# LLNL/saamge

Hardware: AMD Instinct MI355X
Metric: AMG setup+solve DoF/s (3D Poisson, PCG to 1e-8) (higher is better)
Workload: dtype f64; 1 GPU; 3D Poisson 256^3 Q1 hexes, 3-level SAAMGE, theta=0.003, nu_relax=3, 8x8x4-element AEs, 8x8x4-AE coarse blocks; workload_id=poisson256, dofs=16974593, converged=True, parallelism=single GPU

## Files before the change

### saamge_amd/csrc/mis.hip

```cpp
#include "mis.h"
#include "assemble.h"

#include <cfloat>

namespace saamge_amd {

__device__ inline double wsum(double v) {
#pragma unroll
    for (int o = 32; o > 0; o >>= 1) v += __shfl_xor(v, o, 64);
    return v;
}

__global__ __launch_bounds__(64) void mis_svd_kernel(
    const int *__restrict__ mis2d_I, const int *__restrict__ mis2d_J,
    const int *__restrict__ mis2ae_I, const int *__restrict__ mis2ae_J,
    const int *__restrict__ ae2d_I, const int64_t *__restrict__ pair_loc_off,
    const int *__restrict__ pair_loc, const signed char *__restrict__ flags, MisSvdIO io, int m0,
    const int *__restrict__ list = nullptr) {
    extern __shared__ __align__(16) double lds[];
    const int m = list ? list[blockIdx.x] : m0 + (int)blockIdx.x;
    const int lane = threadIdx.x;
    const int r = mis2d_I[m + 1] - mis2d_I[m];
    const int *dofs = mis2d_J + mis2d_I[m];
    double *M = io.gather + io.g_off[m];
// ... 309 lines not shown
        hipLaunchKernelGGL(mis_copy_kernel, dim3(div_up(nm, 4)), dim3(256), 0, s, v, nm, rep.p);
        SA_HIP_CHECK(hipGetLastError());
        SA_HIP_CHECK(hipStreamSynchronize(s));
        profiler().end(s, "mis_svd", 0.0, 0.0);
        return;
    }
    profiler().begin(s);
    hipLaunchKernelGGL(mis_svd_kernel, dim3(num_mises), dim3(64), lds, s, rel.mis2d_I.p,
                       rel.mis2d_J.p, rel.mis2ae_I.p, rel.mis2ae_J.p, rel.ae2d_I.p,
                       rel.pair_loc_off.p, rel.pair_loc.p, rel.flags.p, io, m0);
    SA_HIP_CHECK(hipGetLastError());
    profiler().end(s, "mis_svd", 0.0, 0.0);
}

__global__ __launch_bounds__(256) void p_count_kernel(int ND, const int *__restrict__ mises,
                                                      const int *__restrict__ k, int *__restrict__ cnt) {
    const long i = (long)blockIdx.x * 256 + threadIdx.x;
    if (i < ND) cnt[i] = k[mises[i]];
}

__global__ __launch_bounds__(256) void r_len_kernel(int nm, const int *__restrict__ mis2d_I, const int *__restrict__ k,
                                                    const int *__restrict__ coloff, int *__restrict__ len) {
    const int m = blockIdx.x * 256 + threadIdx.x;
    if (m >= nm) return;
    const int r = mis2d_I[m + 1] - mis2d_I[m], c0 = coloff[m];
    for (int v = 0; v < k[m]; ++v) len[c0 + v] = r;
}

template <class OUT>
__global__ __launch_bounds__(256) void scan_tile_kernel(int n, const int *__restrict__ in,
                                                        OUT *__restrict__ out, OUT *__restrict__ tsum) {
    __shared__ OUT sh[256];
    const long base = (long)blockIdx.x * 1024;
    int v[4];
    OUT run = 0;
    for (int q = 0; q < 4; ++q) {
        const long i = base + threadIdx.x * 4 + q;
        v[q] = (i < n) ? in[i] : 0;
        run += v[q];
    }
    sh[threadIdx.x] = run;
    __syncthreads();
    for (int o = 1; o < 256; o <<= 1) {
        const OUT t = (threadIdx.x >= o) ? sh[threadIdx.x - o] : 0;
        __syncthreads();
        sh[threadIdx.x] += t;
        __syncthreads();
    }
    OUT excl = sh[threadIdx.x] - run;
    for (int q = 0; q < 4; ++q) {
        const long i = base + threadIdx.x * 4 + q;
        if (i < n) out[i] = excl;
        excl += v[q];
    }
    if (threadIdx.x == 255) tsum[blockIdx.x] = sh[255];
}
template <class OUT>
__global__ __launch_bounds__(256) void scan_sums_kernel(int nt, OUT *__restrict__ tsum, OUT *__restrict__ total) {
    __shared__ OUT sh[256];
    __shared__ OUT carry;
    if (threadIdx.x == 0) carry = 0;
    __syncthreads();
    for (int base = 0; base < nt; base += 256) {
        const int i = base + threadIdx.x;
        const OUT x = (i < nt) ? tsum[i] : 0;
        sh[threadIdx.x] = x;
        __syncthreads();
        for (int o = 1; o < 256; o <<= 1) {
            const OUT t = (threadIdx.x >= o) ? sh[threadIdx.x - o] : 0;
            __syncthreads();
            sh[threadIdx.x] += t;
            __syncthreads();
        }
        if (i < nt) tsum[i] = carry + sh[threadIdx.x] - x;
        __syncthreads();
        if (threadIdx.x == 255) carry += sh[255];
        __syncthreads();
    }
    if (threadIdx.x == 0) *total = carry;
}
template <class OUT>
__global__ __launch_bounds__(256) void scan_add_kernel(int n, OUT *__restrict__ out,
                                                       const OUT *__restrict__ tsum,
                                                       const OUT *__restrict__ total) {
    const long i = (long)blockIdx.x * 256 + threadIdx.x;
    if (i < n) out[i] += tsum[i >> 10];
    if (i == 0) out[n] = *total;
}

template <class OUT>
static void exclusive_scan_t(hipStream_t s, int n, const int *in, OUT *out) {
    const int nt = div_up(n, 1024);
    DBuf<OUT> tsum((size_t)nt + 1);
    hipLaunchKernelGGL(scan_tile_kernel<OUT>, dim3(nt), dim3(256), 0, s, n, in, out, tsum.p);
    hipLaunchKernelGGL(scan_sums_kernel<OUT>, dim3(1), dim3(256), 0, s, nt, tsum.p, tsum.p + nt);
    hipLaunchKernelGGL(scan_add_kernel<OUT>, dim3(div_up(n, 256)), dim3(256), 0, s, n, out, (const OUT *)tsum.p, (const OUT *)(tsum.p + nt));
    SA_HIP_CHECK(hipGetLastError());
    SA_HIP_CHECK(hipStreamSynchronize(s));
}
void exclusive_scan_int(hipStream_t s, int n, const int *in, int *out) { exclusive_scan_t<int>(s, n, in, out); }
void exclusive_scan_int_async(hipStream_t s, int n, const int *in, int *out, int *tsum) {
    const int nt = div_up(n, 1024);
    hipLaunchKernelGGL(scan_tile_kernel<int>, dim3(nt), dim3(256), 0, s, n, in, out, tsum);
    hipLaunchKernelGGL(scan_sums_kernel<int>, dim3(1), dim3(256), 0, s, nt, tsum, tsum + nt);
    hipLaunchKernelGGL(scan_add_kernel<int>, dim3(div_up(n, 256)), dim3(256), 0, s, n, out, (const int *)tsum, (const int *)(tsum + nt));
    SA_HIP_CHECK(hipGetLastError());
}
void exclusive_scan_off(hipStream_t s, int n, const int *in, roff_t *out) { exclusive_scan_t<roff_t>(s, n, in, out); }

__global__ __launch_bounds__(256) void p_fill_kernel(int ND, const int *__restrict__ mises,
                                                     const int *__restrict__ row_in_mis,
                                                     const int *__restrict__ mis2d_I,
                                                     const int *__restrict__ k,
                                                     const int *__restrict__ coloff,
                                                     const int64_t *__restrict__ u_off,
                                                     const double *__restrict__ U,
                                                     const roff_t *__restrict__ rowptr,
                                                     int *__restrict__ col, double *__restrict__ val) {
    const long i = (long)blockIdx.x * 256 + threadIdx.x;
    if (i >= ND) return;
    const int m = mises[i], km = k[m];
    const int r = mis2d_I[m + 1] - mis2d_I[m];
    const double *Um = U + u_off[m] + row_in_mis[i];
    const roff_t base = rowptr[i];
    const int c0 = coloff[m];
    for (int v = 0; v < km; ++v) {
        col[base + v] = c0 + v;
        val[base + v] = Um[(size_t)v * r];
    }
}

__global__ __launch_bounds__(256) void r_fill_kernel(int num_mises, const int *__restrict__ mis2d_I,
                                                     const int *__restrict__ mis2d_J,
                                                     const int *__restrict__ k,
                                                     const int *__restrict__ coloff,
                                                     const int64_t *__restrict__ u_off,
                                                     const double *__restrict__ U,
                                                     const roff_t *__restrict__ rowptr,
                                                     int *__restrict__ col, double *__restrict__ val) {
    const int m = blockIdx.x;
    const int km = k[m];
    if (km == 0) return;
    const int r = mis2d_I[m + 1] - mis2d_I[m];
    const int *dofs = mis2d_J + mis2d_I[m];
    const double *Um = U + u_off[m];
    for (int idx = threadIdx.x; idx < km * r; idx += 256) {
        const int v = idx / r, i = idx % r;
        const roff_t base = rowptr[coloff[m] + v];
        col[base + i] = dofs[i];
        val[base + i] = Um[(size_t)v * r + i];
    }
}

void build_P_R(hipStream_t s, const DevRelations &rel, const Relations &hrel,
               const std::vector<int> &h_k, const std::vector<int64_t> &h_u_off, const int *d_k,
               const int *d_coloff, const int64_t *d_u_off, const double *U, DCsr &P, DCsr &R) {
    (void)h_u_off;
    const int ND = hrel.ND;
    int nc = 0;
    int64_t nnz = 0;
    for (int m = 0; m < hrel.num_mises; ++m) {
        nc += h_k[m];
        nnz += (int64_t)h_k[m] * hrel.mis_to_dof.row_size(m);
    }
    P.nrows = ND; P.ncols = nc; P.nnz = nnz;
    P.rowptr.alloc((size_t)ND + 1);
    P.col.alloc((size_t)nnz);
    P.val.alloc((size_t)nnz);
    {
        DBuf<int> cnt((size_t)ND);
        hipLaunchKernelGGL(p_count_kernel, dim3(div_up(ND, 256)), dim3(256), 0, s, ND, rel.mises.p, d_k, cnt.p);
        exclusive_scan_off(s, ND, cnt.p, P.rowptr.p);
    }
    hipLaunchKernelGGL(p_fill_kernel, dim3(div_up(ND, 256)), dim3(256), 0, s, ND, rel.mises.p,
                       rel.dof_row_in_mis.p, rel.mis2d_I.p, d_k, d_coloff, d_u_off, U, P.rowptr.p,
                       P.col.p, P.val.p);
    P.lanes_per_row = pick_lanes_per_row(nnz, ND);
    R.nrows = nc; R.ncols = ND; R.nnz = nnz;
    {
        DBuf<int> len((size_t)std::max(nc, 1));
        R.rowptr.alloc((size_t)nc + 1);
        if (hrel.num_mises)
            hipLaunchKernelGGL(r_len_kernel, dim3(div_up(hrel.num_mises, 256)), dim3(256), 0, s, hrel.num_mises, rel.mis2d_I.p, d_k,
                               d_coloff, len.p);
        if (nc > 0) exclusive_scan_off(s, nc, len.p, R.rowptr.p);
        else SA_HIP_CHECK(hipMemsetAsync(R.rowptr.p, 0, sizeof(roff_t), s));
    }
    R.col.alloc((size_t)nnz);
    R.val.alloc((size_t)nnz);
    if (hrel.num_mises)
        hipLaunchKernelGGL(r_fill_kernel, dim3(hrel.num_mises), dim3(256), 0, s, hrel.num_mises,
                           rel.mis2d_I.p, rel.mis2d_J.p, d_k, d_coloff, d_u_off, U, R.rowptr.p,
                           R.col.p, R.val.p);
    SA_HIP_CHECK(hipGetLastError());
    R.lanes_per_row = pick_lanes_per_row(nnz, nc > 0 ? nc : 1);
}

__global__ __launch_bounds__(256) void ae_mis_k_kernel(long n, const int *__restrict__ ae2mis_J,
                                                       const int *__restrict__ k, int *__restrict__ out) {
    const long i = (long)blockIdx.x * 256 + threadIdx.x;
    if (i < n) out[i] = k[ae2mis_J[i]];
}

__global__ __launch_bounds__(256) void ae_ke_max_kernel(int nparts, const int *__restrict__ ae2mis_I,
                                                        const int *__restrict__ colpos_ptr, int *__restrict__ out) {
    const int e = blockIdx.x * 256 + threadIdx.x;
    int ke = 0;
    if (e < nparts) ke = colpos_ptr[ae2mis_I[e + 1]] - colpos_ptr[ae2mis_I[e]];
#pragma unroll
    for (int o = 32; o > 0; o >>= 1) ke = max(ke, __shfl_xor(ke, o, 64));
    if ((threadIdx.x & 63) == 0) atomicMax(out, ke);
}

__global__ __launch_bounds__(256) void coarse_e2d_kernel(
    const int *__restrict__ ae2d_I, const int *__restrict__ ae2d_J, const int *__restrict__ ae2mis_I,
    const int *__restrict__ ae2mis_J, const int *__restrict__ mises, const int *__restrict__ mis_k,
    const int *__restrict__ mis_coloff, const int *__restrict__ colpos_ptr, const roff_t *__restrict__ prow,
    const double *__restrict__ pval, int cap, int *__restrict__ colpos, int *__restrict__ e2d_J,
    int *__restrict__ err) {
    extern __shared__ unsigned long long ce_keys[];
    int *cd = (int *)(ce_keys + cap);
    const int e = blockIdx.x, tid = threadIdx.x;
    const int tb = ae2mis_I[e], te = ae2mis_I[e + 1];
    const int c0 = colpos_ptr[tb], KE = colpos_ptr[te] - c0;
    for (int t = tb + tid; t < te; t += 256) {
        const int m = ae2mis_J[t], km = mis_k[m], base = colpos_ptr[t] - c0, co = mis_coloff[m];
        for (int v = 0; v < km; ++v) {
            ce_keys[base + v] = ~0ull;
            cd[base + v] = co + v;
        }
    }
    __syncthreads();
    const int d0 = ae2d_I[e], d1 = ae2d_I[e + 1];
    for (int k = d0 + tid; k < d1; k += 256) {
        const int dof = ae2d_J[k], m = mises[dof], km = mis_k[m];
        if (km == 0) continue;
        int lo = tb, hi = te;
        while (lo < hi) {
            const int mid = (lo + hi) >> 1;
            if (ae2mis_J[mid] < m) lo = mid + 1; else hi = mid;
        }
        const int base = colpos_ptr[lo] - c0;
        const roff_t pr = prow[dof];
        for (int v = 0; v < km; ++v)
            if (pval[pr + v] != 0.0)
                atomicMin(&ce_keys[base + v], ((unsigned long long)(unsigned)(k - d0) << 32) | (unsigned)(base + v));
    }
    __syncthreads();
    for (int idx = tid; idx < KE; idx += 256) {
        const unsigned long long key = ce_keys[idx];
        if (key == ~0ull) {
            colpos[c0 + idx] = -1;
            atomicExch(err, 1);
            continue;
        }
        int rank = 0;
        for (int j = 0; j < KE; ++j) rank += (ce_keys[j] < key) ? 1 : 0;
        colpos[c0 + idx] = rank;
        e2d_J[c0 + rank] = cd[idx];
    }
}

bool coarse_e2d_device(hipStream_t s, const DevRelations &rel, const Relations &hrel, const int *d_mis_k,
                       const int *d_mis_coloff, int ncoarse, const roff_t *p_rowptr, const double *p_val,
                       DBuf<int> &colpos_ptr, DBuf<int> &colpos, Table &e2d) {
    const int nparts = hrel.nparts;
    const long npairs = (long)hrel.AE_to_mis.J.size();
    if (nparts == 0 || npairs == 0) return false;
    DBuf<int> kk((size_t)npairs), info(2);
    info.zero(s);
    hipLaunchKernelGGL(ae_mis_k_kernel, dim3(div_up(npairs, 256)), dim3(256), 0, s, npairs, rel.ae2mis_J.p, d_mis_k, kk.p);
    colpos_ptr.alloc((size_t)npairs + 1);
    exclusive_scan_int(s, (int)npairs, kk.p, colpos_ptr.p);
    hipLaunchKernelGGL(ae_ke_max_kernel, dim3(div_up(nparts, 256)), dim3(256), 0, s, nparts, rel.ae2mis_I.p, colpos_ptr.p, info.p);
    SA_HIP_CHECK(hipGetLastError());
    const int cap = info.to_host(s)[0];
    const size_t lds = (size_t)cap * 12 + 16;
    if (lds > 60 * 1024) return false;
    auto h_ptr = colpos_ptr.to_host(s);
    const int total = h_ptr[(size_t)npairs];
    colpos.alloc((size_t)total + 1);
    DBuf<int> d_J((size_t)total + 1);
    if (total) {
        hipLaunchKernelGGL(coarse_e2d_kernel, dim3(nparts), dim3(256), lds, s, rel.ae2d_I.p, rel.ae2d_J.p, rel.ae2mis_I.p,
                           rel.ae2mis_J.p, rel.mises.p, d_mis_k, d_mis_coloff, colpos_ptr.p, p_rowptr, p_val, cap, colpos.p,
                           d_J.p, info.p + 1);
        SA_HIP_CHECK(hipGetLastError());
    }
    SA_REQUIRE(info.to_host(s)[1] == 0, "coarse dof with an all-zero prolongator column in an AE");
    e2d.ncols = ncoarse;
    e2d.I.resize((size_t)nparts + 1);
    for (int e = 0; e <= nparts; ++e) e2d.I[e] = h_ptr[(size_t)hrel.AE_to_mis.I[e]];
    e2d.J.resize((size_t)total);
    if (total) {
        SA_HIP_CHECK(hipMemcpyAsync(e2d.J.data(), d_J.p, sizeof(int) * (size_t)total, hipMemcpyDeviceToHost, s));
        SA_HIP_CHECK(hipStreamSynchronize(s));
    }
    return true;
}

constexpr int RAP_NT = 256;
constexpr int RAP_HASH = 2048;
constexpr int RAP_SMALL_ROWS = 64;

template <int NT, int CAP>
__global__ __launch_bounds__(NT) void rap_symbolic_kernel(
    const int *__restrict__ mlist, int pass, const int *__restrict__ mis2d_I, const int *__restrict__ mis2d_J,
    const roff_t *__restrict__ Arow, const int *__restrict__ Acol, const int *__restrict__ mises,
    const int *__restrict__ k, int *__restrict__ cnt, const int *__restrict__ nbr_ptr,
    int *__restrict__ nbr, int *__restrict__ err, int *__restrict__ stage = nullptr, int stage_cap = 0,
    int maxrow = 0) {
    __shared__ int table[CAP];
    __shared__ int nfound;
    const int m1 = mlist ? mlist[blockIdx.x] : (int)blockIdx.x;
    if (k[m1] == 0) {
        if (pass == 0 && threadIdx.x == 0) cnt[m1] = 0;
        return;
    }
    const int r1 = mis2d_I[m1 + 1] - mis2d_I[m1];
    const int *dofs = mis2d_J + mis2d_I[m1];
    __shared__ int overflow;
    int HS = CAP;
    if (maxrow > 0) {
        const long bound = 2l * r1 * maxrow;
        HS = 64;
        while (HS < 256 && HS < bound) HS <<= 1;
    }
    const bool certain = maxrow > 0 && 2l * r1 * maxrow <= HS;
    for (;;) {
        for (int i = threadIdx.x; i < HS; i += NT) table[i] = -1;
        if (threadIdx.x == 0) { nfound = 0; overflow = 0; }
        __syncthreads();
        for (int il = threadIdx.x; il < r1; il += NT) {
            const int g = dofs[il];
            for (roff_t q = Arow[g]; q < Arow[g + 1]; ++q) {
                const int m2 = mises[Acol[q]];
                if (k[m2] == 0) continue;
                unsigned h = hash_home((unsigned)m2, (unsigned)HS);
                for (int probe = 0; probe < HS; ++probe) {
                    const int old = atomicCAS(&table[h], -1, m2);
                    if (old == -1) { atomicAdd(&nfound, 1); break; }
                    if (old == m2) break;
                    h = (h + 1) & (HS - 1);
                    if (probe == HS - 1) { if (HS == RAP_HASH) atomicExch(err, 1); else overflow = 1; }
                }
            }
        }
        __syncthreads();
        const bool full = !certain && (overflow || 2 * nfound > HS);
        const bool again = HS < CAP && full;
        __syncthreads();
        if (CAP < RAP_HASH && full && !again) {
            if (threadIdx.x == 0) cnt[m1] = -1;
            return;
        }
        if (!again) break;
        HS = CAP;
    }
    if (pass == 0) {
        if (threadIdx.x == 0) cnt[m1] = nfound;
        if (!stage || nfound > stage_cap) return;
    }
    __shared__ int list[CAP];
    __shared__ int nlist;
    if (threadIdx.x == 0) nlist = 0;
    __syncthreads();
    for (int i = threadIdx.x; i < HS; i += NT) {
        const int v = table[i];
        if (v >= 0) list[atomicAdd(&nlist, 1)] = v;
    }
    __syncthreads();
    const int nl = nlist;
    int *out = (pass == 0) ? stage + (size_t)m1 * stage_cap : nbr + nbr_ptr[m1];
    for (int i = threadIdx.x; i < nl; i += NT) {
        const int v = list[i];
        int rank = 0;
        for (int j = 0; j < nl; ++j) rank += (list[j] < v);
        out[rank] = v;
    }
}

__global__ __launch_bounds__(256) void rap_unstage_kernel(int nm, int cap, const int *__restrict__ stage,
                                                          const int *__restrict__ nbr_ptr, int *__restrict__ nbr) {
    const long i = (long)blockIdx.x * 256 + threadIdx.x;
    const int m = (int)(i / cap), t = (int)(i % cap);
    if (m < nm && t < nbr_ptr[m + 1] - nbr_ptr[m]) nbr[nbr_ptr[m] + t] = stage[i];
}

template <int NT>
__global__ __launch_bounds__(NT) void rap_numeric_kernel(
    const int *__restrict__ list, int m_first, const int *__restrict__ mis2d_I, const int *__restrict__ mis2d_J, const roff_t *__restrict__ Arow,
    const int *__restrict__ Acol, const double *__restrict__ Aval, const int *__restrict__ mises,
    const int *__restrict__ row_in_mis, const int *__restrict__ k, const int *__restrict__ coloff,
    const int64_t *__restrict__ u_off, const double *__restrict__ U,
    const int *__restrict__ nbr_ptr, const int *__restrict__ nbr, const roff_t *__restrict__ crowptr,
    int *__restrict__ ccol, double *__restrict__ cval, int lds_doubles) {
    extern __shared__ __align__(16) double lds[];
    const int m1 = list ? list[blockIdx.x] : m_first + (int)blockIdx.x;
    const int k1 = k[m1];
    if (k1 == 0) return;
    const int tid = threadIdx.x;
    const int nn = nbr_ptr[m1 + 1] - nbr_ptr[m1];
    const int *nb = nbr + nbr_ptr[m1];
    const int r1 = mis2d_I[m1 + 1] - mis2d_I[m1];
    const int *dofs = mis2d_J + mis2d_I[m1];
    const double *U1 = U + u_off[m1];
    const int pos_d = 3 * nn + 2;
    long long *uo = (long long *)lds;
    int *pos = (int *)(uo + nn);
    int *nbl = pos + nn + 1;
    int *kk = nbl + nn;
    int *rr = kk + nn;
    for (int t = tid; t < nn; t += NT) {
        const int m2 = nb[t];
        nbl[t] = m2;
        kk[t] = k[m2];
        rr[t] = mis2d_I[m2 + 1] - mis2d_I[m2];
        uo[t] = u_off[m2];
    }
    __syncthreads();
    if (tid == 0) {
        int run = 0;
        for (int t = 0; t < nn; ++t) { pos[t] = run; run += kk[t]; }
        pos[nn] = run;
    }
    __syncthreads();
    const int ncol = pos[nn];
    double *acc = lds + pos_d;
    const int rows_total = (lds_doubles - pos_d) / ncol;
    const int KC = (k1 + 1 <= rows_total) ? k1 : rows_total / 2;
    const int RC = rows_total - KC;
    double *T = acc + (size_t)KC * ncol;
    for (int idx = tid; idx < k1 * ncol; idx += NT) {
        const int v1 = idx / ncol, cc = idx % ncol;
        int lo = 0, hi = nn;
        while (hi - lo > 1) { const int mid = (lo + hi) >> 1; if (pos[mid] <= cc) lo = mid; else hi = mid; }
        ccol[crowptr[coloff[m1] + v1] + cc] = coloff[nbl[lo]] + (cc - pos[lo]);
    }
    for (int v0 = 0; v0 < k1; v0 += KC) {
        const int kc = min(KC, k1 - v0);
        __syncthreads();
        for (int i = tid; i < kc * ncol; i += NT) acc[i] = 0.0;
        for (int c0 = 0; c0 < r1; c0 += RC) {
            const int rc = min(RC, r1 - c0);
            __syncthreads();
            for (int i = tid; i < rc * ncol; i += NT) T[i] = 0.0;
            __syncthreads();
            for (int il = tid; il < rc; il += NT) {
                const int g = dofs[c0 + il];
                double *Trow = T + (size_t)il * ncol;
                const roff_t qe = Arow[g + 1];
                for (roff_t q0 = Arow[g]; q0 < qe; q0 += 4) {
                    int jj4[4], lo4[4];
                    double a4[4], u4[4];
                    bool on4[4];
#pragma unroll
                    for (int t = 0; t < 4; ++t) {
                        const roff_t q = min(q0 + t, qe - 1);
                        jj4[t] = Acol[q];
                        a4[t] = Aval[q];
                    }
                    int m4[4], rim4[4];
#pragma unroll
                    for (int t = 0; t < 4; ++t) { m4[t] = mises[jj4[t]]; rim4[t] = row_in_mis[jj4[t]]; }
#pragma unroll
                    for (int t = 0; t < 4; ++t) {
                        int lo = 0, hi = nn;
                        while (hi - lo > 1) { const int mid = (lo + hi) >> 1; if (nbl[mid] <= m4[t]) lo = mid; else hi = mid; }
                        lo4[t] = lo;
                        on4[t] = q0 + t < qe && nn != 0 && nbl[lo] == m4[t];
                        u4[t] = on4[t] ? U[uo[lo] + rim4[t]] : 0.0;
                    }
#pragma unroll
                    for (int t = 0; t < 4; ++t) {
                        if (!on4[t]) continue;
                        const int lo = lo4[t];
                        const int k2 = kk[lo];
                        const int r2 = rr[lo];
                        const double *U2 = U + uo[lo] + rim4[t];
                        double *dst = Trow + pos[lo];
                        dst[0] = fma(a4[t], u4[t], dst[0]);
                        for (int v = 1; v < k2; ++v) dst[v] = fma(a4[t], U2[(size_t)v * r2], dst[v]);
                    }
                }
            }
            __syncthreads();
            for (int idx = tid; idx < kc * ncol; idx += NT) {
                const int v1 = idx / ncol, cc = idx % ncol;
                double sum = acc[idx];
                const double *u = U1 + (size_t)(v0 + v1) * r1 + c0;
                for (int il = 0; il < rc; ++il) sum = fma(u[il], T[(size_t)il * ncol + cc], sum);
                acc[idx] = sum;
            }
        }
        __syncthreads();
        for (int idx = tid; idx < kc * ncol; idx += NT) {
            const int v1 = idx / ncol, cc = idx % ncol;
            cval[crowptr[coloff[m1] + v0 + v1] + cc] = acc[idx];
        }
    }
}

void rap_mis(hipStream_t s, const DevRelations &rel, const Relations &hrel, const DCsr &A,
             const std::vector<int> &h_k, const std::vector<int> &h_coloff, const int *d_k,
             const int *d_coloff, const int64_t *d_u_off, const double *U, DCsr &Ac, int rank, int world,
             std::vector<long long> *nnz_off) {
    const int nm = hrel.num_mises;
    int nc = 0;
    for (int m = 0; m < nm; ++m) nc += h_k[m];
    Ac.nrows = Ac.ncols = nc;
    Ac.nnz = 0;
    if (nm == 0 || nc == 0) {
        Ac.rowptr.from_host(std::vector<roff_t>(1, 0), s);
        return;
    }
    DBuf<int> cnt((size_t)nm), err(1);
    err.zero(s);
    if (A.max_row < 0) A.max_row = csr_max_row(s, A);
    const int maxrow = A.max_row;
    profiler().begin(s);
    constexpr int STAGE_CAP = 64;
    DBuf<int> stage((size_t)nm * STAGE_CAP);
    {
        std::vector<int> sym_small, sym_big;
        for (int m = 0; m < nm; ++m) (hrel.mis_to_dof.row_size(m) <= RAP_SMALL_ROWS ? sym_small : sym_big).push_back(m);
        DBuf<int> d_sym_small, d_sym_big;
        d_sym_small.from_host(sym_small, s);
        d_sym_big.from_host(sym_big, s);
        if (!sym_big.empty())
            hipLaunchKernelGGL((rap_symbolic_kernel<RAP_NT, RAP_HASH>), dim3((unsigned)sym_big.size()), dim3(RAP_NT), 0, s, d_sym_big.p, 0,
                               rel.mis2d_I.p, rel.mis2d_J.p, A.rowptr.p, A.col.p, rel.mises.p, d_k, cnt.p, nullptr, nullptr, err.p, stage.p,
                               STAGE_CAP, maxrow);
        if (!sym_small.empty())
            hipLaunchKernelGGL((rap_symbolic_kernel<64, 256>), dim3((unsigned)sym_small.size()), dim3(64), 0, s, d_sym_small.p, 0,
                               rel.mis2d_I.p, rel.mis2d_J.p, A.rowptr.p, A.col.p, rel.mises.p, d_k, cnt.p, nullptr, nullptr, err.p, stage.p,
                               STAGE_CAP, maxrow);
        SA_HIP_CHECK(hipGetLastError());
        SA_HIP_CHECK(hipStreamSynchronize(s));
    }
    auto h_cnt = cnt.to_host(s);
    {
        std::vector<int> again;
        for (int m = 0; m < nm; ++m)
            if (h_cnt[m] < 0) again.push_back(m);
        if (!again.empty()) {
            DBuf<int> d_again;
            d_again.from_host(again, s);
            hipLaunchKernelGGL((rap_symbolic_kernel<RAP_NT, RAP_HASH>), dim3((unsigned)again.size()), dim3(RAP_NT), 0, s, d_again.p, 0,
                               rel.mis2d_I.p, rel.mis2d_J.p, A.rowptr.p, A.col.p, rel.mises.p, d_k, cnt.p, nullptr, nullptr, err.p, stage.p,
                               STAGE_CAP, maxrow);
            SA_HIP_CHECK(hipGetLastError());
            h_cnt = cnt.to_host(s);
        }
    }
    SA_REQUIRE(err.to_host(s)[0] == 0, "RAP: MIS neighbour table overflow");
    std::vector<int> h_nbr_ptr((size_t)nm + 1, 0);
    int cnt_max = 0;
    for (int m = 0; m < nm; ++m) { h_nbr_ptr[m + 1] = h_nbr_ptr[m] + h_cnt[m]; cnt_max = std::max(cnt_max, (int)h_cnt[m]); }
    DBuf<int> nbr_ptr, nbr((size_t)h_nbr_ptr[nm] + 1);
    nbr_ptr.from_host(h_nbr_ptr, s);
    if (cnt_max <= STAGE_CAP)
        hipLaunchKernelGGL(rap_unstage_kernel, dim3(div_up((long)nm * STAGE_CAP, 256)), dim3(256), 0, s, nm, STAGE_CAP, stage.p,
                           nbr_ptr.p, nbr.p);
    else
        hipLaunchKernelGGL((rap_symbolic_kernel<RAP_NT, RAP_HASH>), dim3(nm), dim3(RAP_NT), 0, s, (const int *)nullptr, 1, rel.mis2d_I.p,
                           rel.mis2d_J.p, A.rowptr.p, A.col.p, rel.mises.p, d_k, cnt.p, nbr_ptr.p, nbr.p, err.p, (int *)nullptr, 0,
                           maxrow);
    SA_HIP_CHECK(hipGetLastError());
    auto h_nbr = nbr.to_host(s);
    std::vector<roff_t> crow((size_t)nc + 1, 0);
    int64_t nnz = 0;
    size_t need_max = 0, small_max = 0;
    std::vector<int> small_need((size_t)nm, 0);
    for (int m = 0; m < nm; ++m) {
        if (h_k[m] == 0) continue;
        int ncol = 0;
        for (int t = h_nbr_ptr[m]; t < h_nbr_ptr[m + 1]; ++t) ncol += h_k[h_nbr[t]];
        for (int v = 0; v < h_k[m]; ++v) {
            crow[(size_t)h_coloff[m] + v + 1] = ncol;
            nnz += ncol;
        }
        size_t need = (size_t)(3 * h_cnt[m] + 2) + (size_t)(h_k[m] + 1) * ncol;
        const size_t cap = 160 * 1024 / 8;
        if (need > cap) need = std::max((size_t)(3 * h_cnt[m] + 2) + 2 * (size_t)ncol, std::min(need, cap));
        if (need > need_max) need_max = need;
        small_max = std::max(small_max, (size_t)(3 * h_cnt[m] + 2) + (size_t)(h_k[m] + 8) * ncol);
        {
            const size_t tables = (size_t)(3 * h_cnt[m] + 2);
            const size_t all = tables + (size_t)(h_k[m] + hrel.mis_to_dof.row_size(m)) * ncol, floor8 = tables + (size_t)(h_k[m] + 8) * ncol;
            small_need[m] = (int)std::min<size_t>(std::min(all, std::max((size_t)1024, floor8)), 1u << 30);
        }
    }
    for (int i = 0; i < nc; ++i) crow[i + 1] += crow[i];
    size_t lds_doubles = std::max((size_t)2048, small_max);
    if (need_max > 8192) lds_doubles = need_max;
    SA_REQUIRE(lds_doubles * 8 <= 160 * 1024, "RAP: MIS block too wide for LDS");
    SA_HIP_CHECK(hipFuncSetAttribute((const void *)rap_numeric_kernel<RAP_NT>, hipFuncAttributeMaxDynamicSharedMemorySize, 160 * 1024));
    SA_HIP_CHECK(hipFuncSetAttribute((const void *)rap_numeric_kernel<64>, hipFuncAttributeMaxDynamicSharedMemorySize, 160 * 1024));
    Ac.nnz = nnz;
    Ac.rowptr.from_host(crow, s);
    Ac.col.alloc((size_t)nnz);
    Ac.val.alloc((size_t)nnz);
    int m_lo = 0, m_hi = nm;
    if (world > 1 && nnz_off) {
        std::vector<int> mb((size_t)world + 1, nm);
        mb[0] = 0;
        int r = 0;
        for (int m = 0; m < nm && r + 1 < world; ++m) {
            const int64_t done = crow[(size_t)h_coloff[m + 1]];
            while (r + 1 < world && done >= nnz * (r + 1) / world) mb[++r] = m + 1;
        }
        mb[world] = nm;
        nnz_off->assign((size_t)world + 1, 0);
        for (int q = 0; q <= world; ++q) (*nnz_off)[q] = crow[(size_t)h_coloff[mb[q]]];
        m_lo = mb[rank];
        m_hi = mb[rank + 1];
    }
    std::vector<int> small_list, big_list;
    size_t small_lds = 0;
    for (int m = m_lo; m < m_hi; ++m) {
        if (h_k[m] == 0) continue;
        if (hrel.mis_to_dof.row_size(m) <= RAP_SMALL_ROWS && small_need[m] <= 2048) {
            small_list.push_back(m);
            small_lds = std::max(small_lds, (size_t)small_need[m]);
        } else big_list.push_back(m);
    }
    DBuf<int> d_small, d_big;
    d_small.from_host(small_list, s);
    d_big.from_host(big_list, s);
    if (!big_list.empty())
        hipLaunchKernelGGL(rap_numeric_kernel<RAP_NT>, dim3((unsigned)big_list.size()), dim3(RAP_NT), lds_doubles * 8, s, d_big.p, 0,
                           rel.mis2d_I.p, rel.mis2d_J.p, A.rowptr.p, A.col.p, A.val.p, rel.mises.p,
                           rel.dof_row_in_mis.p, d_k, d_coloff, d_u_off, U, nbr_ptr.p, nbr.p, Ac.rowptr.p,
                           Ac.col.p, Ac.val.p, (int)lds_doubles);
    if (!small_list.empty()) {
        const size_t sl = std::max((size_t)256, small_lds);
        hipLaunchKernelGGL(rap_numeric_kernel<64>, dim3((unsigned)small_list.size()), dim3(64), sl * 8, s, d_small.p, 0,
                           rel.mis2d_I.p, rel.mis2d_J.p, A.rowptr.p, A.col.p, A.val.p, rel.mises.p,
                           rel.dof_row_in_mis.p, d_k, d_coloff, d_u_off, U, nbr_ptr.p, nbr.p, Ac.rowptr.p,
                           Ac.col.p, Ac.val.p, (int)sl);
    }
    SA_HIP_CHECK(hipGetLastError());
    SA_HIP_CHECK(hipStreamSynchronize(s));
    profiler().end(s, "rap", 12.0 * (double)(A.nnz + nnz) + 4.0 * A.nrows, 0.0);
    Ac.lanes_per_row = pick_lanes_per_row(nnz, nc);
}

}
```

Baseline: 68.57 million DoF/s.

## Move RAP symbolic bookkeeping to device and pack per-dof MIS lookups

Replaces the host loops in the MIS-based RAP (list classification, counts, row pointers, LDS sizing) with small device kernels plus scans and compaction, so large nbr/cnt arrays no longer travel to the host. Packs mises, row_in_mis and the k==0 flag into one 64-bit word per dof, so the symbolic and numeric kernels do one gather instead of three. The symbolic kernel now spreads the nonzeros of 64-row chunks evenly across threads using a prefix sum, instead of assigning one row per thread. In exchange it adds several small kernel launches and extra host syncs for the compaction sizes.

New measurement: 69.79 million DoF/s (median of 6 runs). 1.8% higher.

```diff
diff --git a/saamge_amd/csrc/mis.hip b/saamge_amd/csrc/mis.hip
--- a/saamge_amd/csrc/mis.hip
+++ b/saamge_amd/csrc/mis.hip
@@ -635,16 +635,60 @@
 constexpr int RAP_NT = 256;
 constexpr int RAP_HASH = 2048;
 constexpr int RAP_SMALL_ROWS = 64;
+constexpr int RAP_SUB = 64;
+constexpr int RAP_ROW_CLAMP = 1 << 24;
+
+typedef unsigned long long rap_word_t;
+constexpr rap_word_t RAP_K0 = 1ull << 63;
+__global__ __launch_bounds__(256) void rap_pack_kernel(int n, const int *__restrict__ mises, const int *__restrict__ row_in_mis,
+                                                       const int *__restrict__ k, rap_word_t *__restrict__ pack) {
+    const long i = (long)blockIdx.x * 256 + threadIdx.x;
+    if (i >= n) return;
+    const int m = mises[i];
+    pack[i] = (rap_word_t)(unsigned)m | ((rap_word_t)(unsigned)row_in_mis[i] << 32) | (k[m] == 0 ? RAP_K0 : 0ull);
+}
+
+__device__ inline void rap_row_prefix(int nr, const int *__restrict__ dofs, const roff_t *__restrict__ Arow, int clamp,
+                                      int *pre, roff_t *qs) {
+    if (threadIdx.x >= 64) return;
+    const int l = threadIdx.x;
+    int len = 0;
+    if (l < nr) {
+        const int g = dofs[l];
+        const roff_t q0 = Arow[g], n = Arow[g + 1] - q0;
+        len = n < (roff_t)clamp ? (int)n : clamp;
+        qs[l] = q0;
+    }
+    int inc = len;
+#pragma unroll
+    for (int o = 1; o < 64; o <<= 1) {
+        const int t = __shfl_up(inc, o, 64);
+        if (l >= o) inc += t;
+    }
+    if (l < nr) pre[l + 1] = inc;
+    if (l == 0) pre[0] = 0;
+}
+
+__device__ inline int rap_entry_row(const int *pre, int ra, int rb, int base, int e) {
+    int lo = ra, hi = rb;
+    while (hi - lo > 1) {
+        const int mid = (lo + hi) >> 1;
+        if (pre[mid] - base <= e) lo = mid; else hi = mid;
+    }
+    return lo;
+}
 
 template <int NT, int CAP>
 __global__ __launch_bounds__(NT) void rap_symbolic_kernel(
     const int *__restrict__ mlist, int pass, const int *__restrict__ mis2d_I, const int *__restrict__ mis2d_J,
-    const roff_t *__restrict__ Arow, const int *__restrict__ Acol, const int *__restrict__ mises,
+    const roff_t *__restrict__ Arow, const int *__restrict__ Acol, const rap_word_t *__restrict__ pack,
     const int *__restrict__ k, int *__restrict__ cnt, const int *__restrict__ nbr_ptr,
     int *__restrict__ nbr, int *__restrict__ err, int *__restrict__ stage = nullptr, int stage_cap = 0,
     int maxrow = 0) {
     __shared__ int table[CAP];
     __shared__ int nfound;
+    __shared__ roff_t qs[RAP_SUB];
+    __shared__ int pre[RAP_SUB + 1];
     const int m1 = mlist ? mlist[blockIdx.x] : (int)blockIdx.x;
     if (k[m1] == 0) {
         if (pass == 0 && threadIdx.x == 0) cnt[m1] = 0;
@@ -664,11 +708,16 @@
         for (int i = threadIdx.x; i < HS; i += NT) table[i] = -1;
         if (threadIdx.x == 0) { nfound = 0; overflow = 0; }
         __syncthreads();
-        for (int il = threadIdx.x; il < r1; il += NT) {
-            const int g = dofs[il];
-            for (roff_t q = Arow[g]; q < Arow[g + 1]; ++q) {
-                const int m2 = mises[Acol[q]];
-                if (k[m2] == 0) continue;
+        for (int s0 = 0; s0 < r1; s0 += RAP_SUB) {
+            const int nr = min(RAP_SUB, r1 - s0);
+            rap_row_prefix(nr, dofs + s0, Arow, RAP_ROW_CLAMP, pre, qs);
+            __syncthreads();
+            const int ne = pre[nr];
+            for (int e = threadIdx.x; e < ne; e += NT) {
+                const int row = rap_entry_row(pre, 0, nr, 0, e);
+                const rap_word_t w = pack[Acol[qs[row] + (e - pre[row])]];
+                if (w & RAP_K0) continue;
+                const int m2 = (int)(unsigned)w;
                 unsigned h = hash_home((unsigned)m2, (unsigned)HS);
                 for (int probe = 0; probe < HS; ++probe) {
                     const int old = atomicCAS(&table[h], -1, m2);
@@ -678,8 +727,8 @@
                     if (probe == HS - 1) { if (HS == RAP_HASH) atomicExch(err, 1); else overflow = 1; }
                 }
             }
-        }
-        __syncthreads();
+            __syncthreads();
+        }
         const bool full = !certain && (overflow || 2 * nfound > HS);
         const bool again = HS < CAP && full;
         __syncthreads();
@@ -720,11 +769,52 @@
     if (m < nm && t < nbr_ptr[m + 1] - nbr_ptr[m]) nbr[nbr_ptr[m] + t] = stage[i];
 }
 
+__device__ inline void rap_walk_row(roff_t qb, roff_t qe, const int *__restrict__ Acol, const double *__restrict__ Aval,
+                                    const rap_word_t *__restrict__ pack, const double *__restrict__ U, int nn,
+                                    const int *nbl, const long long *uo, const int *kk, const int *rr, const int *pos,
+                                    double *Trow) {
+    for (roff_t q0 = qb; q0 < qe; q0 += 4) {
+        int jj4[4], lo4[4], rim4[4];
+        double a4[4], u4[4];
+        bool on4[4];
+        rap_word_t w4[4];
+#pragma unroll
+        for (int t = 0; t < 4; ++t) {
+            const roff_t q = min(q0 + t, qe - 1);
+            jj4[t] = Acol[q];
+            a4[t] = Aval[q];
+        }
+#pragma unroll
+        for (int t = 0; t < 4; ++t) w4[t] = pack[jj4[t]];
+#pragma unroll
+        for (int t = 0; t < 4; ++t) {
+            const int m = (int)(unsigned)w4[t];
+            rim4[t] = (int)((w4[t] >> 32) & 0x7fffffffu);
+            int lo = 0, hi = nn;
+            while (hi - lo > 1) { const int mid = (lo + hi) >> 1; if (nbl[mid] <= m) lo = mid; else hi = mid; }
+            lo4[t] = lo;
+            on4[t] = q0 + t < qe && nn != 0 && !(w4[t] & RAP_K0) && nbl[lo] == m;
+            u4[t] = on4[t] ? U[uo[lo] + rim4[t]] : 0.0;
+        }
+#pragma unroll
+        for (int t = 0; t < 4; ++t) {
+            if (!on4[t]) continue;
+            const int lo = lo4[t];
+            const int k2 = kk[lo];
+            const int r2 = rr[lo];
+            const double *U2 = U + uo[lo] + rim4[t];
+            double *dst = Trow + pos[lo];
+            dst[0] = fma(a4[t], u4[t], dst[0]);
+            for (int v = 1; v < k2; ++v) dst[v] = fma(a4[t], U2[(size_t)v * r2], dst[v]);
+        }
+    }
+}
+
 template <int NT>
 __global__ __launch_bounds__(NT) void rap_numeric_kernel(
     const int *__restrict__ list, int m_first, const int *__restrict__ mis2d_I, const int *__restrict__ mis2d_J, const roff_t *__restrict__ Arow,
-    const int *__restrict__ Acol, const double *__restrict__ Aval, const int *__restrict__ mises,
-    const int *__restrict__ row_in_mis, const int *__restrict__ k, const int *__restrict__ coloff,
+    const int *__restrict__ Acol, const double *__restrict__ Aval, const rap_word_t *__restrict__ pack,
+    const int *__restrict__ k, const int *__restrict__ coloff,
     const int64_t *__restrict__ u_off, const double *__restrict__ U,
     const int *__restrict__ nbr_ptr, const int *__restrict__ nbr, const roff_t *__restrict__ crowptr,
     int *__restrict__ ccol, double *__restrict__ cval, int lds_doubles) {
@@ -781,41 +871,7 @@
             __syncthreads();
             for (int il = tid; il < rc; il += NT) {
                 const int g = dofs[c0 + il];
-                double *Trow = T + (size_t)il * ncol;
-                const roff_t qe = Arow[g + 1];
-                for (roff_t q0 = Arow[g]; q0 < qe; q0 += 4) {
-                    int jj4[4], lo4[4];
-                    double a4[4], u4[4];
-                    bool on4[4];
-#pragma unroll
-                    for (int t = 0; t < 4; ++t) {
-                        const roff_t q = min(q0 + t, qe - 1);
-                        jj4[t] = Acol[q];
-                        a4[t] = Aval[q];
-                    }
-                    int m4[4], rim4[4];
-#pragma unroll
-                    for (int t = 0; t < 4; ++t) { m4[t] = mises[jj4[t]]; rim4[t] = row_in_mis[jj4[t]]; }
-#pragma unroll
-                    for (int t = 0; t < 4; ++t) {
-                        int lo = 0, hi = nn;
-                        while (hi - lo > 1) { const int mid = (lo + hi) >> 1; if (nbl[mid] <= m4[t]) lo = mid; else hi = mid; }
-                        lo4[t] = lo;
-                        on4[t] = q0 + t < qe && nn != 0 && nbl[lo] == m4[t];
-                        u4[t] = on4[t] ? U[uo[lo] + rim4[t]] : 0.0;
-                    }
-#pragma unroll
-                    for (int t = 0; t < 4; ++t) {
-                        if (!on4[t]) continue;
-                        const int lo = lo4[t];
-                        const int k2 = kk[lo];
-                        const int r2 = rr[lo];
-                        const double *U2 = U + uo[lo] + rim4[t];
-                        double *dst = Trow + pos[lo];
-                        dst[0] = fma(a4[t], u4[t], dst[0]);
-                        for (int v = 1; v < k2; ++v) dst[v] = fma(a4[t], U2[(size_t)v * r2], dst[v]);
-                    }
-                }
+                rap_walk_row(Arow[g], Arow[g + 1], Acol, Aval, pack, U, nn, nbl, uo, kk, rr, pos, T + (size_t)il * ncol);
             }
             __syncthreads();
             for (int idx = tid; idx < kc * ncol; idx += NT) {
@@ -832,6 +888,104 @@
             cval[crowptr[coloff[m1] + v0 + v1] + cc] = acc[idx];
         }
     }
+}
+
+enum { RAP_SC_AGAIN = 0, RAP_SC_CNT_MAX, RAP_SC_NEED_MAX, RAP_SC_SMALL_MAX, RAP_SC_SMALL_LDS, RAP_NSC };
+
+__global__ __launch_bounds__(256) void rap_sym_class_kernel(int nm, const int *__restrict__ mis2d_I, int *__restrict__ fa,
+                                                            int *__restrict__ fb) {
+    const int m = blockIdx.x * 256 + threadIdx.x;
+    if (m >= nm) return;
+    const int small = mis2d_I[m + 1] - mis2d_I[m] <= RAP_SMALL_ROWS;
+    fa[m] = small;
+    fb[m] = !small;
+}
+
+__global__ __launch_bounds__(256) void rap_cnt_stats_kernel(int nm, const int *__restrict__ cnt, int *__restrict__ fa,
+                                                            unsigned long long *__restrict__ sc) {
+    const int m = blockIdx.x * 256 + threadIdx.x;
+    const int c = m < nm ? cnt[m] : 0;
+    int neg = c < 0, mx = max(c, 0);
+    if (m < nm) fa[m] = neg;
+#pragma unroll
+    for (int o = 32; o > 0; o >>= 1) {
+        neg += __shfl_xor(neg, o, 64);
+        mx = max(mx, __shfl_xor(mx, o, 64));
+    }
+    if ((threadIdx.x & 63) == 0) {
+        if (neg) atomicAdd(&sc[RAP_SC_AGAIN], (unsigned long long)neg);
+        if (mx) atomicMax(&sc[RAP_SC_CNT_MAX], (unsigned long long)mx);
+    }
+}
+
+__global__ __launch_bounds__(256) void rap_size_kernel(int nm, const int *__restrict__ k, const int *__restrict__ coloff,
+                                                       const int *__restrict__ mis2d_I, const int *__restrict__ nbr_ptr,
+                                                       const int *__restrict__ nbr, unsigned long long cap,
+                                                       int *__restrict__ rowlen, int *__restrict__ small_need,
+                                                       unsigned long long *__restrict__ sc) {
+    typedef unsigned long long u64;
+    const int m = blockIdx.x * 256 + threadIdx.x;
+    u64 need = 0, small = 0;
+    if (m < nm) {
+        const int km = k[m];
+        int sn = 0;
+        if (km > 0) {
+            const int t0 = nbr_ptr[m], t1 = nbr_ptr[m + 1];
+            int ncol = 0;
+            for (int t = t0; t < t1; ++t) ncol += k[nbr[t]];
+            for (int v = 0; v < km; ++v) rowlen[coloff[m] + v] = ncol;
+            const u64 tables = (u64)(3 * (t1 - t0) + 2);
+            need = tables + (u64)(km + 1) * ncol;
+            if (need > cap) need = max(tables + 2ull * ncol, min(need, cap));
+            small = tables + (u64)(km + 8) * ncol;
+            const u64 all = tables + (u64)(km + (mis2d_I[m + 1] - mis2d_I[m])) * ncol;
+            sn = (int)min(min(all, max((u64)1024, small)), (u64)(1u << 30));
+        }
+        small_need[m] = sn;
+    }
+#pragma unroll
+    for (int o = 32; o > 0; o >>= 1) {
+        need = max(need, (u64)__shfl_xor((long long)need, o, 64));
+        small = max(small, (u64)__shfl_xor((long long)small, o, 64));
+    }
+    if ((threadIdx.x & 63) == 0) {
+        if (need) atomicMax(&sc[RAP_SC_NEED_MAX], need);
+        if (small) atomicMax(&sc[RAP_SC_SMALL_MAX], small);
+    }
+}
+
+__global__ __launch_bounds__(256) void rap_num_class_kernel(int nm, int m_lo, int m_hi, const int *__restrict__ k,
+                                                            const int *__restrict__ mis2d_I, const int *__restrict__ small_need,
+                                                            int *__restrict__ fa, int *__restrict__ fb,
+                                                            unsigned long long *__restrict__ sc) {
+    const int m = blockIdx.x * 256 + threadIdx.x;
+    int lds = 0;
+    if (m < nm) {
+        const bool on = m >= m_lo && m < m_hi && k[m] > 0;
+        const bool small = on && mis2d_I[m + 1] - mis2d_I[m] <= RAP_SMALL_ROWS && small_need[m] <= 2048;
+        fa[m] = small;
+        fb[m] = on && !small;
+        if (small) lds = small_need[m];
+    }
+#pragma unroll
+    for (int o = 32; o > 0; o >>= 1) lds = max(lds, __shfl_xor(lds, o, 64));
+    if ((threadIdx.x & 63) == 0 && lds) atomicMax(&sc[RAP_SC_SMALL_LDS], (unsigned long long)lds);
+}
+
+__global__ __launch_bounds__(256) void rap_scatter_kernel(int nm, const int *__restrict__ flag, const int *__restrict__ pos,
+                                                          int *__restrict__ list) {
+    const int m = blockIdx.x * 256 + threadIdx.x;
+    if (m < nm && flag[m]) list[pos[m]] = m;
+}
+
+static int rap_compact(hipStream_t s, int nm, const int *flag, int *pos, DBuf<int> &list) {
+    exclusive_scan_int(s, nm, flag, pos);
+    int n = 0;
+    SA_HIP_CHECK(hipMemcpyAsync(&n, pos + nm, sizeof(int), hipMemcpyDeviceToHost, s));
+    SA_HIP_CHECK(hipStreamSynchronize(s));
+    list.alloc((size_t)n);
+    if (n) hipLaunchKernelGGL(rap_scatter_kernel, dim3(div_up(nm, 256)), dim3(256), 0, s, nm, flag, (const int *)pos, list.p);
+    return n;
 }
 
 void rap_mis(hipStream_t s, const DevRelations &rel, const Relations &hrel, const DCsr &A,
@@ -851,91 +1005,82 @@
     err.zero(s);
     if (A.max_row < 0) A.max_row = csr_max_row(s, A);
     const int maxrow = A.max_row;
+    SA_REQUIRE(maxrow <= RAP_ROW_CLAMP, "RAP: a row of A is too long");
     profiler().begin(s);
+    DBuf<rap_word_t> pack((size_t)A.nrows);
+    hipLaunchKernelGGL(rap_pack_kernel, dim3(div_up(A.nrows, 256)), dim3(256), 0, s, A.nrows, rel.mises.p, rel.dof_row_in_mis.p, d_k, pack.p);
     constexpr int STAGE_CAP = 64;
     DBuf<int> stage((size_t)nm * STAGE_CAP);
+    DBuf<int> fa((size_t)nm), fb((size_t)nm), pos((size_t)nm + 1);
+    DBuf<unsigned long long> sc(RAP_NSC);
+    const dim3 gm(div_up(nm, 256));
     {
-        std::vector<int> sym_small, sym_big;
-        for (int m = 0; m < nm; ++m) (hrel.mis_to_dof.row_size(m) <= RAP_SMALL_ROWS ? sym_small : sym_big).push_back(m);
+        hipLaunchKernelGGL(rap_sym_class_kernel, gm, dim3(256), 0, s, nm, rel.mis2d_I.p, fa.p, fb.p);
         DBuf<int> d_sym_small, d_sym_big;
-        d_sym_small.from_host(sym_small, s);
-        d_sym_big.from_host(sym_big, s);
-        if (!sym_big.empty())
-            hipLaunchKernelGGL((rap_symbolic_kernel<RAP_NT, RAP_HASH>), dim3((unsigned)sym_big.size()), dim3(RAP_NT), 0, s, d_sym_big.p, 0,
-                               rel.mis2d_I.p, rel.mis2d_J.p, A.rowptr.p, A.col.p, rel.mises.p, d_k, cnt.p, nullptr, nullptr, err.p, stage.p,
+        const int n_small = rap_compact(s, nm, fa.p, pos.p, d_sym_small), n_big = rap_compact(s, nm, fb.p, pos.p, d_sym_big);
+        if (n_big)
+            hipLaunchKernelGGL((rap_symbolic_kernel<RAP_NT, RAP_HASH>), dim3((unsigned)n_big), dim3(RAP_NT), 0, s, d_sym_big.p, 0,
+                               rel.mis2d_I.p, rel.mis2d_J.p, A.rowptr.p, A.col.p, pack.p, d_k, cnt.p, nullptr, nullptr, err.p, stage.p,
                                STAGE_CAP, maxrow);
-        if (!sym_small.empty())
-            hipLaunchKernelGGL((rap_symbolic_kernel<64, 256>), dim3((unsigned)sym_small.size()), dim3(64), 0, s, d_sym_small.p, 0,
-                               rel.mis2d_I.p, rel.mis2d_J.p, A.rowptr.p, A.col.p, rel.mises.p, d_k, cnt.p, nullptr, nullptr, err.p, stage.p,
+        if (n_small)
+            hipLaunchKernelGGL((rap_symbolic_kernel<64, 256>), dim3((unsigned)n_small), dim3(64), 0, s, d_sym_small.p, 0,
+                               rel.mis2d_I.p, rel.mis2d_J.p, A.rowptr.p, A.col.p, pack.p, d_k, cnt.p, nullptr, nullptr, err.p, stage.p,
                                STAGE_CAP, maxrow);
         SA_HIP_CHECK(hipGetLastError());
         SA_HIP_CHECK(hipStreamSynchronize(s));
     }
-    auto h_cnt = cnt.to_host(s);
-    {
-        std::vector<int> again;
-        for (int m = 0; m < nm; ++m)
-            if (h_cnt[m] < 0) again.push_back(m);
-        if (!again.empty()) {
-            DBuf<int> d_again;
-            d_again.from_host(again, s);
-            hipLaunchKernelGGL((rap_symbolic_kernel<RAP_NT, RAP_HASH>), dim3((unsigned)again.size()), dim3(RAP_NT), 0, s, d_again.p, 0,
-                               rel.mis2d_I.p, rel.mis2d_J.p, A.rowptr.p, A.col.p, rel.mises.p, d_k, cnt.p, nullptr, nullptr, err.p, stage.p,
-                               STAGE_CAP, maxrow);
-            SA_HIP_CHECK(hipGetLastError());
-            h_cnt = cnt.to_host(s);
-        }
-    }
-    SA_REQUIRE(err.to_host(s)[0] == 0, "RAP: MIS neighbour table overflow");
-    std::vector<int> h_nbr_ptr((size_t)nm + 1, 0);
-    int cnt_max = 0;
-    for (int m = 0; m < nm; ++m) { h_nbr_ptr[m + 1] = h_nbr_ptr[m] + h_cnt[m]; cnt_max = std::max(cnt_max, (int)h_cnt[m]); }
-    DBuf<int> nbr_ptr, nbr((size_t)h_nbr_ptr[nm] + 1);
-    nbr_ptr.from_host(h_nbr_ptr, s);
+    sc.zero(s);
+    hipLaunchKernelGGL(rap_cnt_stats_kernel, gm, dim3(256), 0, s, nm, cnt.p, fa.p, sc.p);
+    SA_HIP_CHECK(hipGetLastError());
+    auto h_sc = sc.to_host(s);
+    if (h_sc[RAP_SC_AGAIN]) {
+        DBuf<int> d_again;
+        const int n_again = rap_compact(s, nm, fa.p, pos.p, d_again);
+        hipLaunchKernelGGL((rap_symbolic_kernel<RAP_NT, RAP_HASH>), dim3((unsigned)n_again), dim3(RAP_NT), 0, s, d_again.p, 0,
+                           rel.mis2d_I.p, rel.mis2d_J.p, A.rowptr.p, A.col.p, pack.p, d_k, cnt.p, nullptr, nullptr, err.p, stage.p,
+                           STAGE_CAP, maxrow);
+        sc.zero(s);
+        hipLaunchKernelGGL(rap_cnt_stats_kernel, gm, dim3(256), 0, s, nm, cnt.p, fa.p, sc.p);
+        SA_HIP_CHECK(hipGetLastError());
+        h_sc = sc.to_host(s);
+    }
+    SA_REQUIRE(err.to_host(s)[0] == 0 && h_sc[RAP_SC_AGAIN] == 0, "RAP: MIS neighbour table overflow");
+    const int cnt_max = (int)h_sc[RAP_SC_CNT_MAX];
+    DBuf<int> nbr_ptr((size_t)nm + 1);
+    exclusive_scan_int(s, nm, cnt.p, nbr_ptr.p);
+    int nbr_total = 0;
+    SA_HIP_CHECK(hipMemcpyAsync(&nbr_total, nbr_ptr.p + nm, sizeof(int), hipMemcpyDeviceToHost, s));
+    SA_HIP_CHECK(hipStreamSynchronize(s));
+    DBuf<int> nbr((size_t)nbr_total + 1);
     if (cnt_max <= STAGE_CAP)
         hipLaunchKernelGGL(rap_unstage_kernel, dim3(div_up((long)nm * STAGE_CAP, 256)), dim3(256), 0, s, nm, STAGE_CAP, stage.p,
                            nbr_ptr.p, nbr.p);
     else
         hipLaunchKernelGGL((rap_symbolic_kernel<RAP_NT, RAP_HASH>), dim3(nm), dim3(RAP_NT), 0, s, (const int *)nullptr, 1, rel.mis2d_I.p,
-                           rel.mis2d_J.p, A.rowptr.p, A.col.p, rel.mises.p, d_k, cnt.p, nbr_ptr.p, nbr.p, err.p, (int *)nullptr, 0,
+                           rel.mis2d_J.p, A.rowptr.p, A.col.p, pack.p, d_k, cnt.p, nbr_ptr.p, nbr.p, err.p, (int *)nullptr, 0,
                            maxrow);
+    DBuf<int> rowlen((size_t)nc), small_need((size_t)nm);
+    sc.zero(s);
+    hipLaunchKernelGGL(rap_size_kernel, gm, dim3(256), 0, s, nm, d_k, d_coloff, rel.mis2d_I.p, nbr_ptr.p, nbr.p,
+                       (unsigned long long)(160 * 1024 / 8), rowlen.p, small_need.p, sc.p);
     SA_HIP_CHECK(hipGetLastError());
-    auto h_nbr = nbr.to_host(s);
-    std::vector<roff_t> crow((size_t)nc + 1, 0);
-    int64_t nnz = 0;
-    size_t need_max = 0, small_max = 0;
-    std::vector<int> small_need((size_t)nm, 0);
-    for (int m = 0; m < nm; ++m) {
-        if (h_k[m] == 0) continue;
-        int ncol = 0;
-        for (int t = h_nbr_ptr[m]; t < h_nbr_ptr[m + 1]; ++t) ncol += h_k[h_nbr[t]];
-        for (int v = 0; v < h_k[m]; ++v) {
-            crow[(size_t)h_coloff[m] + v + 1] = ncol;
-            nnz += ncol;
-        }
-        size_t need = (size_t)(3 * h_cnt[m] + 2) + (size_t)(h_k[m] + 1) * ncol;
-        const size_t cap = 160 * 1024 / 8;
-        if (need > cap) need = std::max((size_t)(3 * h_cnt[m] + 2) + 2 * (size_t)ncol, std::min(need, cap));
-        if (need > need_max) need_max = need;
-        small_max = std::max(small_max, (size_t)(3 * h_cnt[m] + 2) + (size_t)(h_k[m] + 8) * ncol);
-        {
-            const size_t tables = (size_t)(3 * h_cnt[m] + 2);
-            const size_t all = tables + (size_t)(h_k[m] + hrel.mis_to_dof.row_size(m)) * ncol, floor8 = tables + (size_t)(h_k[m] + 8) * ncol;
-            small_need[m] = (int)std::min<size_t>(std::min(all, std::max((size_t)1024, floor8)), 1u << 30);
-        }
-    }
-    for (int i = 0; i < nc; ++i) crow[i + 1] += crow[i];
+    Ac.rowptr.alloc((size_t)nc + 1);
+    exclusive_scan_off(s, nc, rowlen.p, Ac.rowptr.p);
+    roff_t nnz = 0;
+    SA_HIP_CHECK(hipMemcpyAsync(&nnz, Ac.rowptr.p + nc, sizeof(roff_t), hipMemcpyDeviceToHost, s));
+    h_sc = sc.to_host(s);
+    const size_t need_max = (size_t)h_sc[RAP_SC_NEED_MAX], small_max = (size_t)h_sc[RAP_SC_SMALL_MAX];
     size_t lds_doubles = std::max((size_t)2048, small_max);
     if (need_max > 8192) lds_doubles = need_max;
     SA_REQUIRE(lds_doubles * 8 <= 160 * 1024, "RAP: MIS block too wide for LDS");
     SA_HIP_CHECK(hipFuncSetAttribute((const void *)rap_numeric_kernel<RAP_NT>, hipFuncAttributeMaxDynamicSharedMemorySize, 160 * 1024));
     SA_HIP_CHECK(hipFuncSetAttribute((const void *)rap_numeric_kernel<64>, hipFuncAttributeMaxDynamicSharedMemorySize, 160 * 1024));
     Ac.nnz = nnz;
-    Ac.rowptr.from_host(crow, s);
     Ac.col.alloc((size_t)nnz);
     Ac.val.alloc((size_t)nnz);
     int m_lo = 0, m_hi = nm;
     if (world > 1 && nnz_off) {
+        const auto crow = Ac.rowptr.to_host(s);
         std::vector<int> mb((size_t)world + 1, nm);
         mb[0] = 0;
         int r = 0;
@@ -949,28 +1094,20 @@
         m_lo = mb[rank];
         m_hi = mb[rank + 1];
     }
-    std::vector<int> small_list, big_list;
-    size_t small_lds = 0;
-    for (int m = m_lo; m < m_hi; ++m) {
-        if (h_k[m] == 0) continue;
-        if (hrel.mis_to_dof.row_size(m) <= RAP_SMALL_ROWS && small_need[m] <= 2048) {
-            small_list.push_back(m);
-            small_lds = std::max(small_lds, (size_t)small_need[m]);
-        } else big_list.push_back(m);
-    }
+    hipLaunchKernelGGL(rap_num_class_kernel, gm, dim3(256), 0, s, nm, m_lo, m_hi, d_k, rel.mis2d_I.p, small_need.p, fa.p, fb.p, sc.p);
     DBuf<int> d_small, d_big;
-    d_small.from_host(small_list, s);
-    d_big.from_host(big_list, s);
-    if (!big_list.empty())
-        hipLaunchKernelGGL(rap_numeric_kernel<RAP_NT>, dim3((unsigned)big_list.size()), dim3(RAP_NT), lds_doubles * 8, s, d_big.p, 0,
-                           rel.mis2d_I.p, rel.mis2d_J.p, A.rowptr.p, A.col.p, A.val.p, rel.mises.p,
-                           rel.dof_row_in_mis.p, d_k, d_coloff, d_u_off, U, nbr_ptr.p, nbr.p, Ac.rowptr.p,
+    const int n_small = rap_compact(s, nm, fa.p, pos.p, d_small), n_big = rap_compact(s, nm, fb.p, pos.p, d_big);
+    const size_t small_lds = (size_t)sc.to_host(s)[RAP_SC_SMALL_LDS];
+    if (n_big)
+        hipLaunchKernelGGL(rap_numeric_kernel<RAP_NT>, dim3((unsigned)n_big), dim3(RAP_NT), lds_doubles * 8, s,
+                           d_big.p, 0, rel.mis2d_I.p, rel.mis2d_J.p, A.rowptr.p, A.col.p, A.val.p, pack.p,
+                           d_k, d_coloff, d_u_off, U, nbr_ptr.p, nbr.p, Ac.rowptr.p,
                            Ac.col.p, Ac.val.p, (int)lds_doubles);
-    if (!small_list.empty()) {
+    if (n_small) {
         const size_t sl = std::max((size_t)256, small_lds);
-        hipLaunchKernelGGL(rap_numeric_kernel<64>, dim3((unsigned)small_list.size()), dim3(64), sl * 8, s, d_small.p, 0,
-                           rel.mis2d_I.p, rel.mis2d_J.p, A.rowptr.p, A.col.p, A.val.p, rel.mises.p,
-                           rel.dof_row_in_mis.p, d_k, d_coloff, d_u_off, U, nbr_ptr.p, nbr.p, Ac.rowptr.p,
+        hipLaunchKernelGGL(rap_numeric_kernel<64>, dim3((unsigned)n_small), dim3(64), sl * 8, s,
+                           d_small.p, 0, rel.mis2d_I.p, rel.mis2d_J.p, A.rowptr.p, A.col.p, A.val.p, pack.p,
+                           d_k, d_coloff, d_u_off, U, nbr_ptr.p, nbr.p, Ac.rowptr.p,
                            Ac.col.p, Ac.val.p, (int)sl);
     }
     SA_HIP_CHECK(hipGetLastError());
```
